# megvii-research/OccDepth

Measured on AMD Instinct MI355X. Metric: frames/sec forward, SemanticKITTI stereo->256x256x32 voxels, higher is better.
Workload: dtype f32 storage and accumulate; matrix arithmetic as 3x bf16 split (hi + mid + lo of both operands, six v_mfma_f32_32x32x16_bf16 per K step; error vs float64 tested within 1.5x of the exact-fp32 kernels', measured 0.8-1.1x) in the head convolutions (K2s3), the small-volume 3x3x3 convolutions and transpo

## Files before the change

### include/occdepth_amd.h

```cpp
#ifndef OCCDEPTH_AMD_H
#define OCCDEPTH_AMD_H

#include <stdint.h>

#ifdef __cplusplus
extern "C" {
#endif

#define OCCD_OK 0
#define OCCD_EINVAL (-1)
#define OCCD_ELAUNCH (-2)
#define OCCD_ENOMEM (-3)

#define OCCD_MAX_VIEWS 4
#define OCCD_MAX_SCALES 4

#define OCCD_ACT_NONE 0
#define OCCD_ACT_RELU 1
#define OCCD_ACT_SIGMOID 2
#define OCCD_ACT_RELU_PRE 3

#define OCCD_ABI_VERSION 22
int occd_abi_version(void);
const char* occd_strerror(int code);
// ... 115 lines not shown
#define OCCD_GEMM_ACT_NONE 0
#define OCCD_GEMM_ACT_SWISH 1
#define OCCD_GEMM_ACT_LEAKY 2
#define OCCD_GEMM_PRE_F16X2 4
typedef struct occd_gemm_args {
    const float* A;
    const float* B;
    float* C;
    const float* bias;
    int32_t M, N, K, batch;
    int64_t lda, ldb, ldc;
    int64_t stride_a, stride_b, stride_c;
    int32_t act;
    float slope;
    int32_t tile_hint;
    int32_t pre;
    const float* res;
    const float* scale_k;
    int32_t act_a;
    const float* bias_n;
    int64_t stride_bias_n;
} occd_gemm_args;
int occd_gemm_f32x3(const occd_gemm_args* a, void* stream);
int occd_gemm_f32x3_splitk_plan(int32_t M, int32_t N, int32_t K, int32_t batch, int32_t* k16_per_z, int32_t* nz,
                                int32_t* row_ranges, int64_t* workspace_floats);
int occd_gemm_f32x3_splitk(const occd_gemm_args* a, int32_t k16_per_z, int32_t nz, int32_t row_ranges, float* workspace,
                           int64_t workspace_floats, void* stream);
int occd_gemm_f32x3_nt(const occd_gemm_args* a, void* stream);
int32_t occd_gemm_f32x3_nt_splits(int32_t M, int32_t N, int32_t K, int32_t batch);
int64_t occd_gemm_x3_packed_elems(int32_t rows, int32_t K);
int occd_gemm_x3_pack(const float* w, void* out, int32_t rows, int32_t K, int64_t ld, int32_t role, int32_t batch,
                      int64_t in_stride, void* stream);
int64_t occd_gemm_f16x2_packed_elems(int32_t rows, int32_t K);
int occd_gemm_f16x2_pack(const float* w, void* out, int32_t rows, int32_t K, int64_t ld, int32_t batch, int64_t in_stride,
                         void* stream);

typedef struct occd_lift_proj_args {
    occd_lift_args lift;
    const double* cam_E;
    const double* cam_k;
    double voxel_size;
    float origin[3];
    int32_t img_w, img_h;
    occd_flosp_args frustum;
    const float* ida;
} occd_lift_proj_args;
int occd_lift_proj_fwd(const occd_lift_proj_args* a, void* stream);

typedef struct occd_lift_bwd_args {
    occd_lift_args fwd;
    const float* gout;
    float* gfeat[OCCD_MAX_SCALES][OCCD_MAX_VIEWS];
    float* gdepth;
} occd_lift_bwd_args;
int occd_lift_bwd(const occd_lift_bwd_args* a, void* stream);

int occd_project_voxels(const double* cam_E_host, const double* cam_k_host, const double* vox_origin_host,
                        double voxel_size, int32_t X, int32_t Y, int32_t Z, int32_t img_w, int32_t img_h,
                        int64_t* pix, uint8_t* fov, float* pix_z, void* stream);

typedef struct occd_vox2pix_args {
    const double* cam_E;
    const double* cam_k;
    const float* ida;
    int64_t* pix;
    uint8_t* fov;
    float* pix_z;
    double vox_origin[3];
    double voxel_size;
    int32_t batch, n_views, X, Y, Z;
    int32_t img_w, img_h;
} occd_vox2pix_args;
int occd_vox2pix(const occd_vox2pix_args* a, void* stream);

int occd_nchw_to_nhwc(const float* in, float* out, int32_t batch, int32_t C,
                      int64_t S, int32_t cs, void* stream);
int occd_nhwc_to_nchw(const float* in, float* out, int32_t batch, int32_t C,
                      int64_t S, int32_t cs, int32_t coff, void* stream);
int occd_softmax_channels(const float* src, float* dst, int64_t rows,
                          int32_t src_cs, int32_t src_coff, int32_t dst_cs,
                          int32_t dst_coff, int32_t n, int32_t dst_pad, void* stream);

int occd_cascade_tail_fwd(const float* part, const float* wn, float* out, int32_t batch, int32_t X,
                          int32_t Y, int32_t Z, int32_t part_cs, int32_t occ_off, int32_t out_cs,
                          int32_t nbr, void* stream);

int occd_affine_act_nchw(const float* x, const float* res, float* y, const float* scale,
                         const float* shift, int32_t batch, int32_t C, int64_t S, int32_t act,
                         float slope, int32_t res_first, void* stream);

int occd_swish_bwd(const float* x, const float* gy, float* gx, int64_t n, void* stream);
int occd_softmax_nchw(const float* x, float* y, int32_t batch, int32_t C, int64_t S, void* stream);
int occd_dwconv2d_nchw(const float* x, const float* w, const float* scale, const float* shift,
                       float* y, int32_t batch, int32_t C, int32_t H, int32_t W, int32_t k,
                       int32_t stride, int32_t pad_top, int32_t pad_left, int32_t Ho, int32_t Wo,
                       int32_t act, void* stream);
int occd_stem_conv3x3_nchw(const float* x, const float* w, const float* scale, const float* shift, float* y,
                           int32_t batch, int32_t H, int32_t W, int32_t cout, int32_t stride, int32_t pad_top,
                           int32_t pad_left, int32_t Ho, int32_t Wo, int32_t act, void* stream);
int occd_upsample_bilinear_cat_nchw(const float* x, const float* skip, float* out, int32_t batch,
                                    int32_t C, int32_t Cskip, int32_t h, int32_t w, int32_t H,
                                    int32_t W, void* stream);
int occd_upsample_bilinear_cat_nhwc(const float* x, const float* skip, float* out, int32_t batch, int32_t C, int32_t Cskip,
                                    int32_t h, int32_t w, int32_t H, int32_t W, void* stream);
int occd_upsample_bilinear_cat_nhwc_rows(const float* x, const float* skip, float* out, int32_t batch, int32_t C, int32_t Cskip,
                                         int32_t h, int32_t w, int32_t H, int32_t W, int32_t out_cs, void* stream);
int occd_upsample_bilinear_nhwc_bwd(const float* gout, float* gx, int32_t batch, int32_t C, int32_t gout_cs, int32_t h,
                                    int32_t w, int32_t H, int32_t W, void* stream);

int occd_upconv_gather_nchw(const float* z, float* out, int32_t batch, int32_t Cout, int32_t h, int32_t w,
                            int32_t H, int32_t W, int64_t z_channel_stride, int64_t z_batch_stride, void* stream);

int occd_upconv_gather_skip_nchw(const float* z, const float* skip, const float* wskip, const float* shift, float* out,
                                 int32_t batch, int32_t Cout, int32_t Cs, int32_t h, int32_t w, int32_t H, int32_t W,
                                 int64_t z_channel_stride, int64_t z_batch_stride, float slope, void* stream);

int occd_wino_input_transform_nchw(const float* x, float* V, int32_t batch, int32_t Cin, int32_t H, int32_t W,
                                   int32_t ty0, int32_t ths, void* stream);
int occd_wino_output_transform_nchw(const float* M, const float* scale, const float* shift, const float* res,
                                    float* y, int32_t batch, int32_t Cout, int32_t H, int32_t W, int32_t ty0,
                                    int32_t ths, int32_t act, float slope, int32_t res_first, void* stream);

typedef struct occd_wino_args {
    const float* x;
    const float* upk;
    const float* shift;
    const float* res;
    float* y;
    int32_t batch, cin, cout, H, W;
    int32_t act, res_first, tile_hint;
    float slope;
} occd_wino_args;
int64_t occd_wino_packed_floats(int32_t cout, int32_t cin);
int occd_wino_pack_weights(const float* w, const float* scale, float* upk, int32_t cout, int32_t cin, void* stream);
int occd_wino_conv3x3_fwd(const occd_wino_args* a, void* stream);

int64_t occd_wino_packed_f16x2_bytes(int32_t cout, int32_t cin);
int occd_wino_pack_weights_f16x2(const float* w, const float* scale, void* upk, int32_t cout, int32_t cin, void* stream);
int occd_wino_conv3x3_f16x2_fwd(const occd_wino_args* a, void* stream);
int occd_wino_conv3x3_f16x2_fwd_ex(const occd_wino_args* a, int32_t max_workgroups, void* stream);

int occd_dwconv2d_bwd_data_nchw(const float* gy, const float* w, float* dx, int32_t batch, int32_t C, int32_t H,
                                int32_t W, int32_t k, int32_t stride, int32_t pad_top, int32_t pad_left, int32_t Ho,
                                int32_t Wo, void* stream);
int64_t occd_dwconv2d_bwd_weight_workspace_floats(int32_t batch, int32_t C, int32_t k, int32_t Ho, int32_t Wo);
int occd_dwconv2d_bwd_weight_nchw(const float* x, const float* gy, float* dw, float* workspace, int32_t batch, int32_t C,
                                  int32_t H, int32_t W, int32_t k, int32_t stride, int32_t pad_top, int32_t pad_left,
                                  int32_t Ho, int32_t Wo, void* stream);
int32_t occd_dwconv2d_pool_blocks(int32_t Ho, int32_t Wo);
int occd_dwconv2d_pool_nchw(const float* x, const float* w, const float* scale, const float* shift, float* y,
                            float* pool_part, int32_t batch, int32_t C, int32_t H, int32_t W, int32_t k,
                            int32_t stride, int32_t pad_top, int32_t pad_left, int32_t Ho, int32_t Wo,
                            int32_t act, int64_t x_plane_stride, void* stream);
int occd_plane_reduce(const float* a, const float* b, float* out, int64_t planes, int64_t S, void* stream);
int occd_se_bwd(const float* gg, const float* gate, const float* sums, const float* r, const float* w_reduce,
                const float* b_reduce, const float* w_expand, float* dz_scratch, float* gm, float* gw_reduce,
                float* gb_reduce, float* gw_expand, float* gb_expand, int32_t batch, int32_t C, int32_t Cr, int64_t S,
                void* stream);
int occd_depthnet_gate(const float* sps, const float* intrins, int64_t intr_stride, float factor, const float* w1,
                       const float* b1, const float* w2, const float* b2, const float* wr, const float* br,
                       const float* we, const float* be, float* gate, int32_t images, int32_t C, void* stream);
int occd_se_gate(const float* pool_part, const float* w_reduce, const float* b_reduce, const float* w_expand,
                 const float* b_expand, float* r_scratch, float* gate, int32_t batch, int32_t C, int32_t Cr,
                 int32_t nblk, int64_t S, void* stream);
int32_t occd_se_gate_set_fused(int32_t on);

int occd_graph_replace_memsets(void* graph);

typedef struct occd_pw_args {
    const float* x;
    const float* wpk;
    const float* shift;
    const float* gate;
    const float* res;
    float* y;
    int64_t N;
    int32_t batch, cin, cout;
    int32_t act, tile_hint;
    float slope;
    int32_t out_nhwc_cs;
} occd_pw_args;
int64_t occd_pw_packed_floats(int32_t cout, int32_t cin);
int occd_pw_pack_weights(const float* w, const float* scale, float* wpk, int32_t cout, int32_t cin, void* stream);
int occd_pw_conv_fwd(const occd_pw_args* a, void* stream);

int occd_argmax_channels(const float* x, int64_t rows, int32_t cs, int32_t coff, int32_t C,
                         const uint16_t* lut, uint16_t* out, void* stream);

#define OCCD_RENDER_MAX_VIEWS 8
typedef struct OccdRenderView {
    float o0[3], ou[3], ov[3];
    float d0[3], du[3], dv[3];
} OccdRenderView;

typedef struct OccdRenderArgs {
    const void* labels;
    const void* target;
    const uint8_t* fov;
    const OccdRenderView* views;
    const uint8_t* palette;
    const uint8_t* background;
    uint8_t* rgb;
    int32_t* hit;
    uint8_t* face;
    float* depth;
    int32_t batch, n_views, H, W;
    int32_t X, Y, Z;
    int32_t label_bytes, target_bytes;
    int32_t n_palette, alpha;
    int32_t view_w[OCCD_RENDER_MAX_VIEWS], view_h[OCCD_RENDER_MAX_VIEWS];
    uint8_t bg_colour[4];
} OccdRenderArgs;
int occd_render_voxels(const OccdRenderArgs* a, void* stream);

typedef struct OccdStereoArgs {
    const float* img;
    uint8_t* gray;
    void* census;
    const float* ida;
    void* workspace;
    uint16_t* S;
    int32_t* d0;
    uint8_t* flags;
    float* disp;
    const double* cam_k;
    const double* cam_E;
    float* depth;
    int32_t batch, H, W, max_disp;
    int32_t p1, p2, uniqueness;
    int32_t ida_views, calib_views;
    float mean[3], std[3];
} OccdStereoArgs;
int64_t occd_stereo_workspace_bytes(int32_t batch, int32_t H, int32_t W, int32_t max_disp);
int occd_stereo_census(const OccdStereoArgs* a, void* stream);
int occd_stereo_sgm(const OccdStereoArgs* a, void* stream);
int occd_stereo_depth(const OccdStereoArgs* a, void* stream);

typedef struct occd_conv3d_wgrad_args {
    const float* x;
    const float* gy;
    float* dw;
    float* workspace;
    int64_t workspace_floats;
    int32_t batch;
    int32_t X, Y, Z, cin, x_cs, x_coff;
    int32_t Xo, Yo, Zo, cout, gy_cs, gy_coff;
    int32_t kx, ky, kz, sx, sy, sz, dx, dy, dz, px, py, pz;
} occd_conv3d_wgrad_args;
int64_t occd_conv3d_wgrad_workspace_floats(const occd_conv3d_wgrad_args* a);
int occd_conv3d_wgrad(const occd_conv3d_wgrad_args* a, void* stream);

typedef struct occd_bn_args {
    const void* x;
    const void* gy;
    const void* y;
    const void* res;
    void* out;
    void* out2;
    const float* a;
    const float* b;
    const float* mean;
    const float* invstd;
    const float* k1;
    const float* k2;
    const float* k3;
    float* partial;
    int64_t rows;
    int64_t S;
    int32_t batch;
    int32_t C, cw;
    int32_t dtype, layout;
    int32_t x_cs, x_coff, gy_cs, gy_coff, y_cs, y_coff, res_cs, res_coff, out_cs, out_coff, out2_cs, out2_coff;
    int32_t act, res_first;
    float slope;
    int32_t nblk;
} occd_bn_args;
int occd_bn_blocks(const occd_bn_args* a);
int occd_bn_stats(const occd_bn_args* a, void* stream);
int occd_bn_stats_combine(const occd_bn_args* a, double* packed, void* stream);
int occd_bn_finish(const double* packed, int32_t C, float eps, float momentum, const float* gamma, const float* beta,
                   float* running_mean, float* running_var, int64_t* num_batches_tracked, float* mean, float* invstd,
                   float* a, float* b, void* stream);
int occd_bn_apply(const occd_bn_args* a, void* stream);
int occd_bn_bwd_reduce(const occd_bn_args* a, void* stream);
int occd_bn_bwd_combine(const float* partial, int32_t nblk, int32_t C, float* packed, void* stream);
int occd_bn_bwd_finish(const float* local, const float* total, int32_t C, const double* packed_fwd, const float* mean,
                       const float* invstd, const float* a, float* k1, float* k2, float* k3, float* gw, float* gb,
                       void* stream);
int occd_bn_bwd_apply(const occd_bn_args* a, void* stream);
int occd_bn_stats_finish(const occd_bn_args* a, double* packed, float eps, float momentum, const float* gamma,
                         const float* beta, float* running_mean, float* running_var, int64_t* num_batches_tracked,
                         float* mean, float* invstd, float* av, float* bv, void* stream);
int occd_bn_bwd_combine_finish(const float* partial, int32_t nblk, int32_t C, const double* packed_fwd, const float* mean,
                               const float* invstd, const float* a, float* k1, float* k2, float* k3, float* gw, float* gb,
                               void* stream);
int occd_bn_small_ok(const occd_bn_args* a);
int occd_bn_fwd_small(const occd_bn_args* a, double* packed, float eps, float momentum, const float* gamma, const float* beta,
                      float* running_mean, float* running_var, int64_t* num_batches_tracked, float* mean, float* invstd,
                      float* av, float* bv, void* stream);
int occd_bn_bwd_small(const occd_bn_args* a, float* gw, float* gb, void* stream);
int64_t occd_bn_xchg_mailbox_bytes(int32_t world, int32_t cmax);
int occd_bn_fwd_small_xchg(const occd_bn_args* a, double* packed, float eps, float momentum, const float* gamma,
                           const float* beta, float* running_mean, float* running_var, int64_t* num_batches_tracked,
                           float* mean, float* invstd, float* av, float* bv, void* const* mailboxes, int32_t rank,
                           int32_t world, int32_t cmax, int32_t timeout_ms, int32_t* status, void* stream);
int occd_bn_bwd_small_xchg(const occd_bn_args* a, const double* packed_fwd, float* gw, float* gb, void* const* mailboxes,
// ... 177 lines not shown
```

### occdepth_amd/csrc/nchw2d.hip

```cpp
#include <cstdlib>
#include "device.h"

namespace {

__global__ void __launch_bounds__(256) affine_act_kernel(const float* __restrict__ x, const float* __restrict__ res,
                                                         float* __restrict__ y, const float* __restrict__ scale,
                                                         const float* __restrict__ shift, int C, long S, int act,
                                                         float slope, int res_first) {
    const int plane = blockIdx.y;
    const int c = plane % C;
    const float s = scale ? scale[c] : 1.f, t = shift ? shift[c] : 0.f;
    const size_t off = (size_t)plane * S;
    const long n4 = ((S & 3) == 0 && ((off & 3) == 0)) ? S >> 2 : 0;
    for (long i = (long)blockIdx.x * 256 + threadIdx.x; i < n4; i += (long)gridDim.x * 256) {
        f32x4 v = *(const f32x4*)(x + off + i * 4);
        v = v * s + t;
        f32x4 r = {0.f, 0.f, 0.f, 0.f};
        if (res) r = *(const f32x4*)(res + off + i * 4);
        if (res_first) v += r;
        v.x = act2d_fast(v.x, act, slope); v.y = act2d_fast(v.y, act, slope);
        v.z = act2d_fast(v.z, act, slope); v.w = act2d_fast(v.w, act, slope);
        if (!res_first) v += r;
        *(f32x4*)(y + off + i * 4) = v;
    }
    for (long i = n4 * 4 + (long)blockIdx.x * 256 + threadIdx.x; i < S; i += (long)gridDim.x * 256) {
        float v = x[off + i] * s + t;
        const float r = res ? res[off + i] : 0.f;
        if (res_first) v += r;
        v = act2d_fast(v, act, slope);
        if (!res_first) v += r;
        y[off + i] = v;
    }
}

template <int K, int STRIDE>
__global__ void __launch_bounds__(256) dwconv2d_direct_kernel(const float* __restrict__ x, const float* __restrict__ w,
                                                              const float* __restrict__ scale, const float* __restrict__ shift,
                                                              float* __restrict__ y, int C, int H, int W, int Ho, int Wo,
                                                              int pad_t, int pad_l, int act, float* __restrict__ pool_part,
                                                              long xps) {
    constexpr int NX = 4, SPAN = (NX - 1) * STRIDE + K;
    __shared__ float wsum[4];
    const int plane = blockIdx.y;
    const int c = plane % C;
    const int wq = (Wo + NX - 1) / NX;
    const int item_raw = blockIdx.x * 256 + threadIdx.x;
    const bool live = item_raw < Ho * wq;
    if (!live && pool_part == nullptr) return;
    const int item = live ? item_raw : 0;
    const int oy = item / wq, ox0 = (item - oy * wq) * NX;
    const float* xp = x + (size_t)plane * xps;
    float wr[K * K];
#pragma unroll
    for (int i = 0; i < K * K; ++i) wr[i] = w[(size_t)c * K * K + i];
    float acc[NX] = {0.f, 0.f, 0.f, 0.f};
    const int ix0 = ox0 * STRIDE - pad_l;
    int cix[SPAN];
    uint32_t cm[SPAN];
#pragma unroll
    for (int j = 0; j < SPAN; ++j) {
        const int ix = ix0 + j;
        cm[j] = 0u - (uint32_t)((unsigned)ix < (unsigned)W);
        cix[j] = min(max(ix, 0), W - 1);
    }
    float v[K][SPAN];
#pragma unroll
    for (int ky = 0; ky < K; ++ky) {
        const int iy = oy * STRIDE - pad_t + ky;
        const uint32_t rm = 0u - (uint32_t)((unsigned)iy < (unsigned)H);
        const float* row = xp + (size_t)min(max(iy, 0), H - 1) * W;
#pragma unroll
        for (int j = 0; j < SPAN; ++j) v[ky][j] = __uint_as_float(__float_as_uint(row[cix[j]]) & (rm & cm[j]));
    }
#pragma unroll
    for (int ky = 0; ky < K; ++ky)
#pragma unroll
        for (int o = 0; o < NX; ++o)
#pragma unroll
            for (int kx = 0; kx < K; ++kx) acc[o] += v[ky][o * STRIDE + kx] * wr[ky * K + kx];
    const float s = scale ? scale[c] : 1.f, t = shift ? shift[c] : 0.f;
    float* yp = y + ((size_t)plane * Ho + oy) * Wo + ox0;
    float part = 0.f;
#pragma unroll
    for (int o = 0; o < NX; ++o)
        if (live && ox0 + o < Wo) {
            const float v = act2d_fast(acc[o] * s + t, act, 0.f);
            yp[o] = v;
            part += v;
        }
    if (pool_part != nullptr) {
#pragma unroll
        for (int off = 32; off > 0; off >>= 1) part += __shfl_down(part, off, 64);
        if ((threadIdx.x & 63) == 0) wsum[threadIdx.x >> 6] = part;
        __syncthreads();
        if (threadIdx.x == 0) pool_part[(size_t)plane * gridDim.x + blockIdx.x] = (wsum[0] + wsum[1]) + (wsum[2] + wsum[3]);
    }
}

template <int K, int STRIDE>
__global__ void __launch_bounds__(256) dwconv2d_kernel(const float* __restrict__ x, const float* __restrict__ w,
                                                       const float* __restrict__ scale, const float* __restrict__ shift,
                                                       float* __restrict__ y, int C, int H, int W, int Ho, int Wo,
                                                       int pad_t, int pad_l, int act, float* __restrict__ pool_part,
                                                       int wp, occd::FastDiv wpd, long xps) {
    constexpr int NX = 4, SPAN = (NX - 1) * STRIDE + K, SPAN4 = (SPAN + 3) / 4;
    extern __shared__ __attribute__((aligned(16))) float tile[];
    __shared__ float wsum[4];
    const int plane = blockIdx.y;
    const int c = plane % C;
    const int wq = (Wo + NX - 1) / NX;
    const int nitems = Ho * wq;
    const int item0 = blockIdx.x * 256;
    const int oy_first = item0 / wq;
    const int oy_last = min(item0 + 255, nitems - 1) / wq;
    const int iy_first = oy_first * STRIDE - pad_t;
    const int nrows = (oy_last - oy_first) * STRIDE + K;
    const float* xp = x + (size_t)plane * xps;
    const int total = nrows * wp;
    for (int e = threadIdx.x; e < total; e += 256) {
        const int r = (int)occd_fastdiv((uint32_t)e, wpd), j = e - r * wp;
        const int iy = iy_first + r, ix = j - pad_l;
        const uint32_t ok = 0u - (uint32_t)(((unsigned)iy < (unsigned)H) & ((unsigned)ix < (unsigned)W));
        const float v = xp[(size_t)min(max(iy, 0), H - 1) * W + min(max(ix, 0), W - 1)];
        tile[e] = __uint_as_float(__float_as_uint(v) & ok);
    }
    float wr[K * K];
#pragma unroll
    for (int i = 0; i < K * K; ++i) wr[i] = w[(size_t)c * K * K + i];
    __syncthreads();
    const int item_raw = item0 + threadIdx.x;
    const bool live = item_raw < nitems;
    const int item = live ? item_raw : item0;
    const int oy = item / wq, q = item - oy * wq, ox0 = q * NX;
    const float* trow = tile + (size_t)((oy - oy_first) * STRIDE) * wp + q * NX * STRIDE;
    float acc[NX] = {0.f, 0.f, 0.f, 0.f};
#pragma unroll
    for (int ky = 0; ky < K; ++ky) {
        float v[SPAN4 * 4];
#pragma unroll
        for (int i = 0; i < SPAN4; ++i) {
            const f32x4 t = *(const f32x4*)(trow + ky * wp + i * 4);
            v[i * 4 + 0] = t.x; v[i * 4 + 1] = t.y; v[i * 4 + 2] = t.z; v[i * 4 + 3] = t.w;
        }
#pragma unroll
        for (int o = 0; o < NX; ++o)
#pragma unroll
            for (int kx = 0; kx < K; ++kx) acc[o] += v[o * STRIDE + kx] * wr[ky * K + kx];
    }
    const float s = scale ? scale[c] : 1.f, t = shift ? shift[c] : 0.f;
    float* yp = y + ((size_t)plane * Ho + oy) * Wo + ox0;
    float part = 0.f;
#pragma unroll
    for (int o = 0; o < NX; ++o)
        if (live && ox0 + o < Wo) {
            const float v = act2d_fast(acc[o] * s + t, act, 0.f);
            yp[o] = v;
            part += v;
        }
    if (pool_part != nullptr) {
#pragma unroll
        for (int off = 32; off > 0; off >>= 1) part += __shfl_down(part, off, 64);
        if ((threadIdx.x & 63) == 0) wsum[threadIdx.x >> 6] = part;
        __syncthreads();
        if (threadIdx.x == 0) pool_part[(size_t)plane * gridDim.x + blockIdx.x] = (wsum[0] + wsum[1]) + (wsum[2] + wsum[3]);
    }
}

template <int K, int STRIDE>
__global__ void __launch_bounds__(256) dwconv2d_bwd_data_kernel(const float* __restrict__ gy, const float* __restrict__ w,
                                                                float* __restrict__ dx, int C, int H, int W, int Ho,
                                                                int Wo, int pad_t, int pad_l) {
    constexpr int NX = 4;
    const int plane = blockIdx.y;
    const int c = plane % C;
    const int wq = (W + NX - 1) / NX;
    const int item = blockIdx.x * 256 + threadIdx.x;
    if (item >= H * wq) return;
    const int iy = item / wq, ix0 = (item - iy * wq) * NX;
    const float* gp = gy + (size_t)plane * Ho * Wo;
    float wr[K * K];
#pragma unroll
    for (int i = 0; i < K * K; ++i) wr[i] = w[(size_t)c * K * K + i];
    float acc[NX] = {0.f, 0.f, 0.f, 0.f};
    if constexpr (STRIDE == 1) {
        constexpr int SP = NX + K - 1;
        const int j0 = ix0 + pad_l - (K - 1);
        int cj[SP];
        uint32_t cm[SP];
#pragma unroll
        for (int j = 0; j < SP; ++j) {
            cm[j] = 0u - (uint32_t)((unsigned)(j0 + j) < (unsigned)Wo);
            cj[j] = min(max(j0 + j, 0), Wo - 1);
        }
        float v[K][SP];
#pragma unroll
        for (int ky = 0; ky < K; ++ky) {
            const int ty = iy + pad_t - ky;
            const uint32_t rm = 0u - (uint32_t)((unsigned)ty < (unsigned)Ho);
            const float* row = gp + (size_t)min(max(ty, 0), Ho - 1) * Wo;
#pragma unroll
            for (int j = 0; j < SP; ++j) v[ky][j] = __uint_as_float(__float_as_uint(row[cj[j]]) & (rm & cm[j]));
        }
#pragma unroll
        for (int ky = 0; ky < K; ++ky)
#pragma unroll
            for (int o = 0; o < NX; ++o)
#pragma unroll
                for (int kx = 0; kx < K; ++kx) acc[o] += v[ky][o + K - 1 - kx] * wr[ky * K + kx];
    } else {
#pragma unroll
        for (int ky = 0; ky < K; ++ky) {
            const int ty = iy + pad_t - ky;
            if (ty < 0 || ty % STRIDE != 0 || ty / STRIDE >= Ho) continue;
            const float* row = gp + (size_t)(ty / STRIDE) * Wo;
#pragma unroll
            for (int o = 0; o < NX; ++o)
#pragma unroll
                for (int kx = 0; kx < K; ++kx) {
                    const int tx = ix0 + o + pad_l - kx;
                    if (tx >= 0 && tx % STRIDE == 0 && tx / STRIDE < Wo) acc[o] += row[tx / STRIDE] * wr[ky * K + kx];
                }
        }
    }
    float* xp = dx + ((size_t)plane * H + iy) * W + ix0;
#pragma unroll
    for (int o = 0; o < NX; ++o)
        if (ix0 + o < W) xp[o] = acc[o];
}

template <int K, int STRIDE>
__global__ void __launch_bounds__(256) dwconv2d_bwd_weight_kernel(const float* __restrict__ x, const float* __restrict__ gy,
                                                                  float* __restrict__ part, int B, int C, int H, int W,
                                                                  int Ho, int Wo, int pad_t, int pad_l) {
    __shared__ float red[4][K * K];
    constexpr int NX = 4, SPAN = (NX - 1) * STRIDE + K;
    const int c = blockIdx.y;
    const int wq = (Wo + NX - 1) / NX;
    const long total = (long)B * Ho * wq;
    float acc[K * K];
#pragma unroll
    for (int i = 0; i < K * K; ++i) acc[i] = 0.f;
    for (long i = (long)blockIdx.x * 256 + threadIdx.x; i < total; i += (long)gridDim.x * 256) {
        const int b = (int)(i / ((long)Ho * wq));
        const int r = (int)(i - (long)b * Ho * wq);
        const int oy = r / wq, ox0 = (r - oy * wq) * NX;
        const float* gp = gy + (((size_t)b * C + c) * Ho + oy) * Wo;
        const float* xp = x + ((size_t)b * C + c) * H * W;
        float g[NX];
#pragma unroll
        for (int o = 0; o < NX; ++o)
            g[o] = __uint_as_float(__float_as_uint(gp[min(ox0 + o, Wo - 1)]) & (0u - (uint32_t)(ox0 + o < Wo)));
        const int ix0 = ox0 * STRIDE - pad_l;
        int cix[SPAN];
        uint32_t cm[SPAN];
#pragma unroll
        for (int j = 0; j < SPAN; ++j) {
            cm[j] = 0u - (uint32_t)((unsigned)(ix0 + j) < (unsigned)W);
            cix[j] = min(max(ix0 + j, 0), W - 1);
        }
        float v[K][SPAN];
#pragma unroll
        for (int ky = 0; ky < K; ++ky) {
            const int iy = oy * STRIDE - pad_t + ky;
            const uint32_t rm = 0u - (uint32_t)((unsigned)iy < (unsigned)H);
            const float* row = xp + (size_t)min(max(iy, 0), H - 1) * W;
#pragma unroll
            for (int j = 0; j < SPAN; ++j) v[ky][j] = __uint_as_float(__float_as_uint(row[cix[j]]) & (rm & cm[j]));
        }
#pragma unroll
        for (int ky = 0; ky < K; ++ky)
#pragma unroll
            for (int kx = 0; kx < K; ++kx)
#pragma unroll
                for (int o = 0; o < NX; ++o) acc[ky * K + kx] += g[o] * v[ky][o * STRIDE + kx];
    }
#pragma unroll
    for (int i = 0; i < K * K; ++i) {
        float v = acc[i];
#pragma unroll
        for (int off = 32; off > 0; off >>= 1) v += __shfl_down(v, off, 64);
        if ((threadIdx.x & 63) == 0) red[threadIdx.x >> 6][i] = v;
    }
    __syncthreads();
    if (threadIdx.x < K * K)
        part[((size_t)c * gridDim.x + blockIdx.x) * (K * K) + threadIdx.x] =
            (red[0][threadIdx.x] + red[1][threadIdx.x]) + (red[2][threadIdx.x] + red[3][threadIdx.x]);
}

__global__ void dwconv2d_bwd_weight_reduce_kernel(const float* __restrict__ part, float* __restrict__ dw, int C, int KK,
                                                  int chunks) {
    const int i = blockIdx.x * blockDim.x + threadIdx.x;
    if (i >= C * KK) return;
    const int c = i / KK, t = i - c * KK;
    float s = 0.f;
    for (int j = 0; j < chunks; ++j) s += part[((size_t)c * chunks + j) * KK + t];
    dw[i] = s;
}

__global__ void __launch_bounds__(256) upsample_cat_kernel(const float* __restrict__ x, const float* __restrict__ skip,
                                                           float* __restrict__ out, int C, int Cs, int h, int w, int H,
                                                           int W, float rh, float rw) {
    const int plane = blockIdx.z;
    const int ct = C + Cs;
    const int b = plane / ct, c = plane - b * ct;
    const int ox0 = (blockIdx.x * 64 + (threadIdx.x & 63)) * 4;
    const int oy = blockIdx.y * 4 + (threadIdx.x >> 6);
    if (ox0 >= W || oy >= H) return;
    float v[4];
    if (c >= C) {
        const float* sp = skip + (((size_t)b * Cs + (c - C)) * H + oy) * W;
#pragma unroll
        for (int i = 0; i < 4; ++i) v[i] = sp[min(ox0 + i, W - 1)];
    } else {
        const float sy = rh * oy;
        const int y0 = (int)sy;
        const int y1 = y0 + (y0 < h - 1);
        const float ly = sy - y0, hy = 1.f - ly;
// ... 293 lines not shown
        const int kx = t % 3;
#pragma unroll
        for (int i = 0; i < 4; ++i) {
            const int j = i + kx;
            acc[i] += cm[j] * ((1.f - lx[j]) * row[x0[j]] + lx[j] * row[x1[j]]);
        }
    }
    }
    if (SKIP) {
        const int lc = ox0 - X0;
#pragma unroll
        for (int c = 0; c < kUpSkipC; ++c) {
            if (c >= sk.Cs) break;
#pragma unroll
            for (int ky = 0; ky < 3; ++ky) {
                const float* srow = S + (c * 6 + r + ky) * kUpSkipW + lc;
                const f32x4 va = *(const f32x4*)srow;
                const f32x2 vb = *(const f32x2*)(srow + 4);
                const float v[6] = {va.x, va.y, va.z, va.w, vb.x, vb.y};
#pragma unroll
                for (int kx = 0; kx < 3; ++kx) {
                    const float wv = wk[(c * 3 + ky) * 3 + kx];
#pragma unroll
                    for (int i = 0; i < 4; ++i) acc[i] += v[i + kx] * wv;
                }
            }
        }
#pragma unroll
        for (int i = 0; i < 4; ++i) {
            const float t = acc[i] + sh;
            acc[i] = t > 0.f ? t : t * sk.slope;
        }
    }
    float* op = out + ((size_t)plane * H + oy) * W + ox0;
    if (ox0 + 3 < W && ((reinterpret_cast<uintptr_t>(op) & 15) == 0)) {
        *(f32x4*)op = f32x4{acc[0], acc[1], acc[2], acc[3]};
    } else {
#pragma unroll
        for (int i = 0; i < 4; ++i)
            if (ox0 + i < W) op[i] = acc[i];
    }
}

}

__global__ void __launch_bounds__(256) softmax_nchw_kernel(const float* __restrict__ x, float* __restrict__ y, int C,
                                                           long S) {
    const long i = (long)blockIdx.x * 256 + threadIdx.x;
    if (i >= S) return;
    const float* xp = x + (size_t)blockIdx.y * C * S + i;
    float* yp = y + (size_t)blockIdx.y * C * S + i;
    float mx = -INFINITY;
    for (int c = 0; c < C; ++c) mx = fmaxf(mx, xp[(size_t)c * S]);
    float sum = 0.f;
    for (int c = 0; c < C; ++c) sum += expf(xp[(size_t)c * S] - mx);
    const float inv = 1.f / sum;
    for (int c = 0; c < C; ++c) yp[(size_t)c * S] = expf(xp[(size_t)c * S] - mx) * inv;
}

__global__ void __launch_bounds__(256) softmax_nchw_c128_kernel(const float* __restrict__ x, float* __restrict__ y, int C,
                                                                long S) {
    __shared__ float red[2][4][64];
    const int lane = threadIdx.x & 63, wave = threadIdx.x >> 6;
    const long i = (long)blockIdx.x * 64 + lane;
    const bool ok = i < S;
    const float* xp = x + (size_t)blockIdx.y * C * S + (ok ? i : S - 1);
    float v[32];
    float mx = -INFINITY;
#pragma unroll
    for (int k = 0; k < 32; ++k) {
        const int c = wave + 4 * k;
        v[k] = c < C ? xp[(size_t)c * S] : -INFINITY;
        mx = fmaxf(mx, v[k]);
    }
    red[0][wave][lane] = mx;
    __syncthreads();
    mx = fmaxf(fmaxf(red[0][0][lane], red[0][1][lane]), fmaxf(red[0][2][lane], red[0][3][lane]));
    float sum = 0.f;
#pragma unroll
    for (int k = 0; k < 32; ++k) {
        v[k] = expf(v[k] - mx);
        sum += v[k];
    }
    red[1][wave][lane] = sum;
    __syncthreads();
    const float inv = 1.f / ((red[1][0][lane] + red[1][1][lane]) + (red[1][2][lane] + red[1][3][lane]));
    if (!ok) return;
    float* yp = y + (size_t)blockIdx.y * C * S + i;
#pragma unroll
    for (int k = 0; k < 32; ++k) {
        const int c = wave + 4 * k;
        if (c < C) yp[(size_t)c * S] = v[k] * inv;
    }
}

extern "C" int occd_softmax_nchw(const float* x, float* y, int32_t batch, int32_t C, int64_t S, void* stream) {
    if (!x || !y || batch <= 0 || batch > 65535 || C <= 0 || S <= 0) return OCCD_EINVAL;
    occd::ProfScope prof("softmax_nchw", (hipStream_t)stream, 0.0, 8.0 * batch * C * (double)S);
    if (C <= 128) {
        hipLaunchKernelGGL(softmax_nchw_c128_kernel, dim3((unsigned)((S + 63) / 64), (unsigned)batch), dim3(256), 0,
                           (hipStream_t)stream, x, y, C, (long)S);
        return occd::check_launch();
    }
    hipLaunchKernelGGL(softmax_nchw_kernel, dim3((unsigned)((S + 255) / 256), (unsigned)batch), dim3(256), 0,
                       (hipStream_t)stream, x, y, C, (long)S);
    return occd::check_launch();
}

__global__ void __launch_bounds__(256) swish_bwd_kernel(const float* __restrict__ x, const float* __restrict__ gy,
                                                        float* __restrict__ gx, long n) {
    const long n4 = n >> 2;
    for (long i = (long)blockIdx.x * 256 + threadIdx.x; i < n4; i += (long)gridDim.x * 256) {
        const f32x4 xv = ((const f32x4*)x)[i], g = ((const f32x4*)gy)[i];
        f32x4 o;
#pragma unroll
        for (int k = 0; k < 4; ++k) {
            const float sg = __builtin_amdgcn_rcpf(1.f + __builtin_amdgcn_exp2f(xv[k] * -1.4426950408889634f));
            o[k] = g[k] * sg * (1.f + xv[k] * (1.f - sg));
        }
        ((f32x4*)gx)[i] = o;
    }
    for (long i = n4 * 4 + (long)blockIdx.x * 256 + threadIdx.x; i < n; i += (long)gridDim.x * 256) {
        const float sg = __builtin_amdgcn_rcpf(1.f + __builtin_amdgcn_exp2f(x[i] * -1.4426950408889634f));
        gx[i] = gy[i] * sg * (1.f + x[i] * (1.f - sg));
    }
}

extern "C" int occd_swish_bwd(const float* x, const float* gy, float* gx, int64_t n, void* stream) {
    if (!x || !gy || !gx || n <= 0) return OCCD_EINVAL;
    if ((reinterpret_cast<uintptr_t>(x) | reinterpret_cast<uintptr_t>(gy) | reinterpret_cast<uintptr_t>(gx)) & 15) return OCCD_EINVAL;
    long blocks = (n / 4 + 255) / 256;
    if (blocks < 1) blocks = 1;
    if (blocks > 8192) blocks = 8192;
    occd::ProfScope prof("swish_bwd", (hipStream_t)stream, 0.0, 12.0 * (double)n);
    hipLaunchKernelGGL(swish_bwd_kernel, dim3((unsigned)blocks), dim3(256), 0, (hipStream_t)stream, x, gy, gx, (long)n);
    return occd::check_launch();
}

extern "C" int occd_affine_act_nchw(const float* x, const float* res, float* y, const float* scale, const float* shift,
                                    int32_t batch, int32_t C, int64_t S, int32_t act, float slope, int32_t res_first,
                                    void* stream) {
    if (!x || !y || batch <= 0 || C <= 0 || S <= 0 || act < 0 || act > 3) return OCCD_EINVAL;
    const long planes = (long)batch * C;
    if (planes > 65535) return OCCD_EINVAL;
    long bx = (S / 4 + 255) / 256;
    if (bx < 1) bx = 1;
    if (bx > 64) bx = 64;
    occd::ProfScope prof("affine_act_nchw", (hipStream_t)stream, 0.0, 4.0 * planes * S * (2 + (res != nullptr)));
    hipLaunchKernelGGL(affine_act_kernel, dim3((unsigned)bx, (unsigned)planes), dim3(256), 0, (hipStream_t)stream, x,
                       res, y, scale, shift, C, (long)S, act, slope, res_first);
    return occd::check_launch();
}

static int dwconv_launch(const float* x, const float* w, const float* scale, const float* shift, float* y,
                         int32_t batch, int32_t C, int32_t H, int32_t W, int32_t k, int32_t stride, int32_t pad_top,
                         int32_t pad_left, int32_t Ho, int32_t Wo, int32_t act, float* pool_part, int64_t x_plane_stride,
                         void* stream) {
    if (!x || !w || !y || batch <= 0 || C <= 0 || H <= 0 || W <= 0 || Ho <= 0 || Wo <= 0 || stride <= 0)
        return OCCD_EINVAL;
    if (x_plane_stride != 0 && x_plane_stride < (int64_t)H * W) return OCCD_EINVAL;
    const long xps = x_plane_stride != 0 ? (long)x_plane_stride : (long)H * W;
    if ((k != 3 && k != 5) || act < 0 || act > 2 || (long)batch * C > 65535) return OCCD_EINVAL;
    if (stride != 1 && stride != 2) return OCCD_EINVAL;
    const int items = Ho * ((Wo + 3) / 4);
    const dim3 grid((unsigned)((items + 255) / 256), (unsigned)(batch * C));
    occd::ProfScope prof("dwconv2d_nchw", (hipStream_t)stream, 2.0 * batch * C * (double)Ho * Wo * k * k,
                         4.0 * batch * C * ((double)H * W + (double)Ho * Wo));
    hipStream_t st = (hipStream_t)stream;
    const int wq = (Wo + 3) / 4;
    const int span4 = ((3 * stride + k) + 3) / 4;
    const int wp = 4 * (wq - 1) * stride + 4 * span4;
    int dmax = (255 + wq - 1) / wq;
    if (dmax > Ho - 1) dmax = Ho - 1;
    const size_t lds = (size_t)(dmax * stride + k) * wp * sizeof(float);
    if (lds <= 48 * 1024) {
#define OCCD_DW(KK, SS)                                                                                             \
    hipLaunchKernelGGL((dwconv2d_kernel<KK, SS>), grid, dim3(256), lds, st, x, w, scale, shift, y, C, H, W, Ho, Wo, \
                       pad_top, pad_left, act, pool_part, wp, occd::make_fastdiv((uint32_t)wp), xps)
        if (k == 3 && stride == 1) OCCD_DW(3, 1);
        else if (k == 3) OCCD_DW(3, 2);
        else if (stride == 1) OCCD_DW(5, 1);
        else OCCD_DW(5, 2);
#undef OCCD_DW
        return occd::check_launch();
    }
#define OCCD_DW(KK, SS)                                                                                                 \
    hipLaunchKernelGGL((dwconv2d_direct_kernel<KK, SS>), grid, dim3(256), 0, st, x, w, scale, shift, y, C, H, W, Ho, Wo, \
                       pad_top, pad_left, act, pool_part, xps)
    if (k == 3 && stride == 1) OCCD_DW(3, 1);
    else if (k == 3) OCCD_DW(3, 2);
    else if (stride == 1) OCCD_DW(5, 1);
    else OCCD_DW(5, 2);
#undef OCCD_DW
    return occd::check_launch();
}

extern "C" int occd_dwconv2d_nchw(const float* x, const float* w, const float* scale, const float* shift, float* y,
                                  int32_t batch, int32_t C, int32_t H, int32_t W, int32_t k, int32_t stride,
                                  int32_t pad_top, int32_t pad_left, int32_t Ho, int32_t Wo, int32_t act,
                                  void* stream) {
    return dwconv_launch(x, w, scale, shift, y, batch, C, H, W, k, stride, pad_top, pad_left, Ho, Wo, act, nullptr, 0, stream);
}

constexpr int kStemCin = 3;
constexpr int kStemRows = 8;
template <int STRIDE>
__global__ void __launch_bounds__(256, 2) stem_conv3x3_kernel(const float* __restrict__ x, const float* __restrict__ w,
                                                           const float* __restrict__ scale, const float* __restrict__ shift,
                                                           float* __restrict__ y, int H, int W, int Cout, int pad_top,
                                                           int pad_left, int Ho, int Wo, int act) {
    extern __shared__ float wl[];
    const int Cout16 = (Cout + 15) & ~15;
    for (int i = threadIdx.x; i < 27 * Cout16; i += 256) {
        const int t = i / Cout16, co = i - t * Cout16;
        wl[i] = co < Cout ? w[co * 27 + t] * (scale != nullptr ? scale[co] : 1.f) : 0.f;
    }
    __syncthreads();
    const int ox = blockIdx.x * 64 + (threadIdx.x & 63);
    const int b = blockIdx.z;
    const int grp = threadIdx.x >> 6;
    if (ox >= Wo) return;
    for (int oy = blockIdx.y * kStemRows; oy < min(Ho, (int)(blockIdx.y + 1) * kStemRows); ++oy) {
    float v[27];
    const float* xb = x + (size_t)b * kStemCin * H * W;
#pragma unroll
    for (int ci = 0; ci < kStemCin; ++ci)
#pragma unroll
        for (int ky = 0; ky < 3; ++ky) {
            const int iy = oy * STRIDE - pad_top + ky;
#pragma unroll
            for (int kx = 0; kx < 3; ++kx) {
                const int ix = ox * STRIDE - pad_left + kx;
                const bool ok = (unsigned)iy < (unsigned)H && (unsigned)ix < (unsigned)W;
                const float t = xb[((size_t)ci * H + min(max(iy, 0), H - 1)) * W + min(max(ix, 0), W - 1)];
                v[ci * 9 + ky * 3 + kx] = ok ? t : 0.f;
            }
        }
    for (int c0 = grp * 16; c0 < Cout16; c0 += 64) {
#pragma unroll 1
        for (int q = 0; q < 4; ++q) {
            f32x4 acc = {0.f, 0.f, 0.f, 0.f};
            const float* wq = wl + c0 + 4 * q;
#pragma unroll
            for (int t0 = 0; t0 < 27; t0 += 9) {
                __builtin_amdgcn_sched_barrier(0);
#pragma unroll
                for (int t = t0; t < t0 + 9; ++t) acc += *(const f32x4*)(wq + t * Cout16) * v[t];
            }
            __builtin_amdgcn_sched_barrier(0);
#pragma unroll
            for (int j = 0; j < 4; ++j) {
                const int co = c0 + 4 * q + j;
                if (co < Cout) {
                    const float o = acc[j] + (shift != nullptr ? shift[co] : 0.f);
                    y[(((size_t)b * Cout + co) * Ho + oy) * Wo + ox] = act2d_fast(o, act, 0.f);
                }
            }
        }
    }
    }
}

extern "C" int occd_stem_conv3x3_nchw(const float* x, const float* w, const float* scale, const float* shift, float* y,
                                      int32_t batch, int32_t H, int32_t W, int32_t cout, int32_t stride, int32_t pad_top,
                                      int32_t pad_left, int32_t Ho, int32_t Wo, int32_t act, void* stream) {
    if (x == nullptr || w == nullptr || y == nullptr) return OCCD_EINVAL;
    if (batch < 1 || batch > 65535 || H < 1 || W < 1 || cout < 1 || cout > 512 || (stride != 1 && stride != 2)) return OCCD_EINVAL;
    if (Ho < 1 || Ho > 65535 || Wo < 1 || pad_top < 0 || pad_left < 0 || act < 0 || act > 2) return OCCD_EINVAL;
    hipStream_t st = (hipStream_t)stream;
    const dim3 grid((unsigned)((Wo + 63) / 64), (unsigned)((Ho + kStemRows - 1) / kStemRows), (unsigned)batch);
    const size_t lds = (size_t)27 * ((cout + 15) & ~15) * sizeof(float);
    occd::ProfScope prof("stem_conv3x3", st, 2.0 * batch * (double)Ho * Wo * 27 * cout,
                         4.0 * batch * ((double)kStemCin * H * W + (double)cout * Ho * Wo));
    if (stride == 2)
        hipLaunchKernelGGL(stem_conv3x3_kernel<2>, grid, dim3(256), lds, st, x, w, scale, shift, y, H, W, cout, pad_top,
                           pad_left, Ho, Wo, act);
    else
        hipLaunchKernelGGL(stem_conv3x3_kernel<1>, grid, dim3(256), lds, st, x, w, scale, shift, y, H, W, cout, pad_top,
                           pad_left, Ho, Wo, act);
    return occd::check_launch();
}

extern "C" int32_t occd_dwconv2d_pool_blocks(int32_t Ho, int32_t Wo) { return (Ho * ((Wo + 3) / 4) + 255) / 256; }

extern "C" int occd_dwconv2d_pool_nchw(const float* x, const float* w, const float* scale, const float* shift, float* y,
                                       float* pool_part, int32_t batch, int32_t C, int32_t H, int32_t W, int32_t k,
                                       int32_t stride, int32_t pad_top, int32_t pad_left, int32_t Ho, int32_t Wo,
                                       int32_t act, int64_t x_plane_stride, void* stream) {
    if (pool_part == nullptr) return OCCD_EINVAL;
    return dwconv_launch(x, w, scale, shift, y, batch, C, H, W, k, stride, pad_top, pad_left, Ho, Wo, act, pool_part,
                         x_plane_stride, stream);
}

__global__ void __launch_bounds__(256) upsample_cat_nhwc_kernel(const float* __restrict__ x, const float* __restrict__ skip,
                                                                float* __restrict__ out, int C, int Cs, int h, int w, int H,
                                                                int W, float rh, float rw, long total, int ct) {
    const long i = (long)blockIdx.x * 256 + threadIdx.x;
    if (i >= total) return;
    const int c = (int)(i % ct);
    long t = i / ct;
    const int ox = (int)(t % W); t /= W;
    const int oy = (int)(t % H);
    const int b = (int)(t / H);
    float v;
    if (c >= C + Cs) {
        v = 0.f;
    } else if (c >= C) {
        v = skip[(((size_t)b * H + oy) * W + ox) * Cs + (c - C)];
    } else {
        const float sy = rh * oy;
        const int y0 = (int)sy;
        const int y1 = y0 + (y0 < h - 1);
        const float ly = sy - y0, hy = 1.f - ly;
        const float sx = rw * ox;
        const int x0 = (int)sx;
        const int x1 = x0 + (x0 < w - 1);
        const float lx = sx - x0, hx = 1.f - lx;
        const float* p0 = x + (((size_t)b * h + y0) * w) * C + c;
        const float* p1 = x + (((size_t)b * h + y1) * w) * C + c;
        v = hy * (hx * p0[(size_t)x0 * C] + lx * p0[(size_t)x1 * C]) + ly * (hx * p1[(size_t)x0 * C] + lx * p1[(size_t)x1 * C]);
    }
    out[i] = v;
}

__global__ void __launch_bounds__(256) upsample_nhwc_bwd_kernel(const float* __restrict__ gout, float* __restrict__ gx, int C,
                                                                int gcs, int h, int w, int H, int W, float rh, float rw,
                                                                float inv_rh, float inv_rw, long total) {
    const long i = (long)blockIdx.x * 256 + threadIdx.x;
    if (i >= total) return;
    const int c = (int)(i % C);
    long t = i / C;
    const int x = (int)(t % w); t /= w;
    const int y = (int)(t % h);
    const int b = (int)(t / h);
    const int Ya = max(0, (int)floorf((y - 1) * inv_rh) - 1), Yb = min(H - 1, (int)ceilf((y + 1) * inv_rh) + 1);
// ... 381 lines not shown
```

Before: 68.19.

## Stage depthwise conv tiles with vector chunk loads and pair small planes per block

Changes the depthwise 2D conv LDS staging from scalar per-element loads to 16-byte chunk loads. Four chunks are batched per thread, and lane shifts with masks handle misaligned edges. When a plane fits in 128 items, two planes share one 256-thread block, which cuts half-empty blocks. Interior outputs are written as a vector store. The aim is fewer global load instructions and better occupancy on small planes, at the cost of extra shift and select logic and a new runtime/env switch.

```diff
diff --git a/include/occdepth_amd.h b/include/occdepth_amd.h
--- a/include/occdepth_amd.h
+++ b/include/occdepth_amd.h
@@ -291,6 +291,7 @@
                             float* pool_part, int32_t batch, int32_t C, int32_t H, int32_t W, int32_t k,
                             int32_t stride, int32_t pad_top, int32_t pad_left, int32_t Ho, int32_t Wo,
                             int32_t act, int64_t x_plane_stride, void* stream);
+int32_t occd_dwconv2d_set_stage(int32_t form);
 int occd_plane_reduce(const float* a, const float* b, float* out, int64_t planes, int64_t S, void* stream);
 int occd_se_bwd(const float* gg, const float* gate, const float* sums, const float* r, const float* w_reduce,
                 const float* b_reduce, const float* w_expand, float* dz_scratch, float* gm, float* gw_reduce,
diff --git a/occdepth_amd/csrc/dwconv_stage.h b/occdepth_amd/csrc/dwconv_stage.h
--- /dev/null
+++ b/occdepth_amd/csrc/dwconv_stage.h
@@ -0,0 +1,67 @@
+#pragma once
+#include <stdint.h>
+
+#if defined(__HIPCC__)
+#define OCCD_DW_HD __host__ __device__ __forceinline__
+#else
+#define OCCD_DW_HD inline
+#endif
+
+namespace occd {
+
+constexpr int kDwPass = 4;
+constexpr int kDwPairItems = 128;
+
+OCCD_DW_HD int dw_tile_wp(int Wo, int k, int stride) {
+    const int wq = (Wo + 3) / 4, span4 = ((3 * stride + k) + 3) / 4;
+    return 4 * (wq - 1) * stride + 4 * span4;
+}
+
+struct DwRows {
+    int oy_first, iy_first, nrows;
+};
+OCCD_DW_HD DwRows dw_tile_rows(int block, int Ho, int Wo, int k, int stride, int pad_t) {
+    const int wq = (Wo + 3) / 4, nitems = Ho * wq, item0 = block * 256;
+    const int last = item0 + 255 < nitems - 1 ? item0 + 255 : nitems - 1;
+    DwRows t;
+    t.oy_first = item0 / wq;
+    t.iy_first = t.oy_first * stride - pad_t;
+    t.nrows = (last / wq - t.oy_first) * stride + k;
+    return t;
+}
+
+OCCD_DW_HD uint32_t dw_div_magic(uint32_t d) { return d <= 1 ? 0u : (uint32_t)((((uint64_t)1 << 32) + d - 1) / d); }
+OCCD_DW_HD uint32_t dw_div(uint32_t n, uint32_t magic) {
+#if defined(__HIP_DEVICE_COMPILE__)
+    return __umulhi(n, magic) + (magic == 0u ? n : 0u);
+#else
+    return (uint32_t)(((uint64_t)n * magic) >> 32) + (magic == 0u ? n : 0u);
+#endif
+}
+
+struct DwChunk {
+    int off, sh;
+    bool row_ok;
+};
+OCCD_DW_HD DwChunk dw_chunk(int f, int wp4, uint32_t wp4_magic, int iy_first, int pad_l, int H, int W) {
+    const int r = (int)dw_div((uint32_t)f, wp4_magic), m = f - r * wp4;
+    const int iy = iy_first + r, ix0 = 4 * m - pad_l;
+    const int cy = iy < 0 ? 0 : iy > H - 1 ? H - 1 : iy;
+    const int cx = ix0 < 0 ? 0 : ix0 > W - 4 ? W - 4 : ix0;
+    DwChunk c;
+    c.off = cy * W + cx;
+    c.sh = ix0 - cx;
+    c.row_ok = (unsigned)iy < (unsigned)H;
+    return c;
+}
+OCCD_DW_HD void dw_shift(const uint32_t u[4], int sh, uint32_t out[4]) {
+    uint32_t eq[7];
+    for (int d = -3; d <= 3; ++d) eq[d + 3] = 0u - (uint32_t)(sh == d);
+    for (int t = 0; t < 4; ++t) {
+        uint32_t v = 0u;
+        for (int i = 0; i < 4; ++i) v |= u[i] & eq[i - t + 3];
+        out[t] = v;
+    }
+}
+
+}
diff --git a/occdepth_amd/csrc/nchw2d.hip b/occdepth_amd/csrc/nchw2d.hip
--- a/occdepth_amd/csrc/nchw2d.hip
+++ b/occdepth_amd/csrc/nchw2d.hip
@@ -1,5 +1,7 @@
+#include <atomic>
 #include <cstdlib>
 #include "device.h"
+#include "dwconv_stage.h"
 
 namespace {
 
@@ -97,16 +99,23 @@
     }
 }
 
-template <int K, int STRIDE>
+typedef float f32x4u __attribute__((ext_vector_type(4), aligned(4)));
+template <int K, int STRIDE, bool CHUNK, bool PAIR = false>
 __global__ void __launch_bounds__(256) dwconv2d_kernel(const float* __restrict__ x, const float* __restrict__ w,
                                                        const float* __restrict__ scale, const float* __restrict__ shift,
                                                        float* __restrict__ y, int C, int H, int W, int Ho, int Wo,
                                                        int pad_t, int pad_l, int act, float* __restrict__ pool_part,
-                                                       int wp, occd::FastDiv wpd, long xps) {
+                                                       int wp, occd::FastDiv wpd, long xps, int planes) {
+    static_assert(CHUNK || !PAIR, "paired planes are a variant of the chunked form");
     constexpr int NX = 4, SPAN = (NX - 1) * STRIDE + K, SPAN4 = (SPAN + 3) / 4;
-    extern __shared__ __attribute__((aligned(16))) float tile[];
+    constexpr int NT = PAIR ? occd::kDwPairItems : 256;
+    extern __shared__ __attribute__((aligned(16))) float tile_all[];
     __shared__ float wsum[4];
-    const int plane = blockIdx.y;
+    const int half = PAIR ? __builtin_amdgcn_readfirstlane((int)threadIdx.x / NT) : 0;
+    const int tid = PAIR ? (int)threadIdx.x % NT : (int)threadIdx.x;
+    const int plane_raw = PAIR ? (int)blockIdx.y * 2 + half : (int)blockIdx.y;
+    const bool pvalid = !PAIR || plane_raw < planes;
+    const int plane = pvalid ? plane_raw : planes - 1;
     const int c = plane % C;
     const int wq = (Wo + NX - 1) / NX;
     const int nitems = Ho * wq;
@@ -116,6 +125,37 @@
     const int iy_first = oy_first * STRIDE - pad_t;
     const int nrows = (oy_last - oy_first) * STRIDE + K;
     const float* xp = x + (size_t)plane * xps;
+    float* const tile = tile_all + (PAIR ? half * nrows * wp : 0);
+    float wr[K * K];
+    if constexpr (CHUNK) {
+#pragma unroll
+        for (int i = 0; i < K * K; ++i) wr[i] = w[(size_t)c * K * K + i];
+    }
+    if constexpr (CHUNK) {
+        const occd::DwRows tr = occd::dw_tile_rows((int)blockIdx.x, Ho, Wo, K, STRIDE, pad_t);
+        const int wp4 = wp >> 2, nchunks = tr.nrows * wp4;
+        for (int base = tid; base < nchunks; base += NT * occd::kDwPass) {
+            f32x4 v[occd::kDwPass];
+#pragma unroll
+            for (int i = 0; i < occd::kDwPass; ++i)
+                v[i] = *(const f32x4u*)(xp + occd::dw_chunk(min(base + i * NT, nchunks - 1), wp4, wpd.magic, tr.iy_first, pad_l, H, W).off);
+#pragma unroll
+            for (int i = 0; i < occd::kDwPass; ++i) {
+                const int f = base + i * NT;
+                if (f >= nchunks) continue;
+                const occd::DwChunk ch = occd::dw_chunk(f, wp4, wpd.magic, tr.iy_first, pad_l, H, W);
+                f32x4 u = v[i];
+                if (ch.sh != 0) {
+                    const uint32_t l[4] = {__float_as_uint(u.x), __float_as_uint(u.y), __float_as_uint(u.z), __float_as_uint(u.w)};
+                    uint32_t o[4];
+                    occd::dw_shift(l, ch.sh, o);
+                    u = f32x4{__uint_as_float(o[0]), __uint_as_float(o[1]), __uint_as_float(o[2]), __uint_as_float(o[3])};
+                }
+                const f32x4 z = {0.f, 0.f, 0.f, 0.f};
+                *(f32x4*)(tile + 4 * f) = ch.row_ok ? u : z;
+            }
+        }
+    } else {
     const int total = nrows * wp;
     for (int e = threadIdx.x; e < total; e += 256) {
         const int r = (int)occd_fastdiv((uint32_t)e, wpd), j = e - r * wp;
@@ -124,13 +164,15 @@
         const float v = xp[(size_t)min(max(iy, 0), H - 1) * W + min(max(ix, 0), W - 1)];
         tile[e] = __uint_as_float(__float_as_uint(v) & ok);
     }
-    float wr[K * K];
-#pragma unroll
-    for (int i = 0; i < K * K; ++i) wr[i] = w[(size_t)c * K * K + i];
+    }
+    if constexpr (!CHUNK) {
+#pragma unroll
+        for (int i = 0; i < K * K; ++i) wr[i] = w[(size_t)c * K * K + i];
+    }
     __syncthreads();
-    const int item_raw = item0 + threadIdx.x;
-    const bool live = item_raw < nitems;
-    const int item = live ? item_raw : item0;
+    const int item_raw = item0 + tid;
+    const bool live = item_raw < nitems && pvalid;
+    const int item = item_raw < nitems ? item_raw : item0;
     const int oy = item / wq, q = item - oy * wq, ox0 = q * NX;
     const float* trow = tile + (size_t)((oy - oy_first) * STRIDE) * wp + q * NX * STRIDE;
     float acc[NX] = {0.f, 0.f, 0.f, 0.f};
@@ -150,6 +192,15 @@
     const float s = scale ? scale[c] : 1.f, t = shift ? shift[c] : 0.f;
     float* yp = y + ((size_t)plane * Ho + oy) * Wo + ox0;
     float part = 0.f;
+    if (CHUNK && live && ox0 + NX - 1 < Wo) {
+        float v[NX];
+#pragma unroll
+        for (int o = 0; o < NX; ++o) {
+            v[o] = act2d_fast(acc[o] * s + t, act, 0.f);
+            part += v[o];
+        }
+        *(f32x4u*)yp = f32x4{v[0], v[1], v[2], v[3]};
+    } else {
 #pragma unroll
     for (int o = 0; o < NX; ++o)
         if (live && ox0 + o < Wo) {
@@ -157,12 +208,17 @@
             yp[o] = v;
             part += v;
         }
+    }
     if (pool_part != nullptr) {
 #pragma unroll
         for (int off = 32; off > 0; off >>= 1) part += __shfl_down(part, off, 64);
         if ((threadIdx.x & 63) == 0) wsum[threadIdx.x >> 6] = part;
         __syncthreads();
+        if constexpr (PAIR) {
+            if (tid == 0 && pvalid) pool_part[(size_t)plane] = (wsum[2 * half] + wsum[2 * half + 1]) + (0.f + 0.f);
+        } else {
         if (threadIdx.x == 0) pool_part[(size_t)plane * gridDim.x + blockIdx.x] = (wsum[0] + wsum[1]) + (wsum[2] + wsum[3]);
+        }
     }
 }
 
@@ -762,6 +818,9 @@
     return occd::check_launch();
 }
 
+static std::atomic<int> g_dw_stage{occd::env_flag("OCCD_DW_STAGE", true) ? 1 : 0};
+extern "C" int32_t occd_dwconv2d_set_stage(int32_t form) { return g_dw_stage.exchange(form < 0 || form > 2 ? 1 : form); }
+
 static int dwconv_launch(const float* x, const float* w, const float* scale, const float* shift, float* y,
                          int32_t batch, int32_t C, int32_t H, int32_t W, int32_t k, int32_t stride, int32_t pad_top,
                          int32_t pad_left, int32_t Ho, int32_t Wo, int32_t act, float* pool_part, int64_t x_plane_stride,
@@ -778,19 +837,30 @@
                          4.0 * batch * C * ((double)H * W + (double)Ho * Wo));
     hipStream_t st = (hipStream_t)stream;
     const int wq = (Wo + 3) / 4;
-    const int span4 = ((3 * stride + k) + 3) / 4;
-    const int wp = 4 * (wq - 1) * stride + 4 * span4;
+    const int wp = occd::dw_tile_wp(Wo, k, stride);
     int dmax = (255 + wq - 1) / wq;
     if (dmax > Ho - 1) dmax = Ho - 1;
     const size_t lds = (size_t)(dmax * stride + k) * wp * sizeof(float);
     if (lds <= 48 * 1024) {
+        const int stage = g_dw_stage.load();
+        const bool chunk = stage != 0 && W >= 4 && (int64_t)H * W <= INT32_MAX;
+        const bool pair = chunk && stage == 1 && items <= occd::kDwPairItems && 2 * lds <= 48 * 1024;
+        const int planes = batch * C;
+        const occd::FastDiv wp4d{occd::dw_div_magic((uint32_t)(wp / 4)), (uint32_t)(wp / 4)};
 #define OCCD_DW(KK, SS)                                                                                             \
-    hipLaunchKernelGGL((dwconv2d_kernel<KK, SS>), grid, dim3(256), lds, st, x, w, scale, shift, y, C, H, W, Ho, Wo, \
-                       pad_top, pad_left, act, pool_part, wp, occd::make_fastdiv((uint32_t)wp), xps)
-        if (k == 3 && stride == 1) OCCD_DW(3, 1);
-        else if (k == 3) OCCD_DW(3, 2);
-        else if (stride == 1) OCCD_DW(5, 1);
-        else OCCD_DW(5, 2);
+    if (pair)                                                                                                       \
+        hipLaunchKernelGGL((dwconv2d_kernel<KK, SS, true, true>), dim3(1, (unsigned)((planes + 1) / 2)), dim3(256), 2 * lds, st, x, w, \
+                           scale, shift, y, C, H, W, Ho, Wo, pad_top, pad_left, act, pool_part, wp, wp4d, xps, planes);  \
+    else if (chunk)                                                                                                 \
+        hipLaunchKernelGGL((dwconv2d_kernel<KK, SS, true>), grid, dim3(256), lds, st, x, w, scale, shift, y, C, H, W, Ho, Wo, \
+                           pad_top, pad_left, act, pool_part, wp, wp4d, xps, planes);                               \
+    else                                                                                                            \
+        hipLaunchKernelGGL((dwconv2d_kernel<KK, SS, false>), grid, dim3(256), lds, st, x, w, scale, shift, y, C, H, W, Ho, Wo, \
+                           pad_top, pad_left, act, pool_part, wp, occd::make_fastdiv((uint32_t)wp), xps, planes)
+        if (k == 3 && stride == 1) { OCCD_DW(3, 1); }
+        else if (k == 3) { OCCD_DW(3, 2); }
+        else if (stride == 1) { OCCD_DW(5, 1); }
+        else { OCCD_DW(5, 2); }
 #undef OCCD_DW
         return occd::check_launch();
     }
```

New measurement: 68.92, median of 6. 1.1% higher.
